# Audio-WestlakeU/SAR-SSL

Hardware: AMD Instinct MI355X
Metric: pretrain_segments_per_sec (higher is better)
Workload: dtype fp16 stem + f32 residual stream (fp16-pair MFMA operands: hi hi + lo hi + hi lo), bf16 backward

## Files before the change

### include/sarssl_hip.h

```cpp
#ifndef SARSSL_HIP_H
#define SARSSL_HIP_H
#ifdef __cplusplus
extern "C" {
#endif

const char* sarssl_last_error(void);
int sarssl_abi_version(void);

typedef struct sarssl_ctx sarssl_ctx;
sarssl_ctx* sarssl_create(int device);
int sarssl_destroy(sarssl_ctx* ctx);
int sarssl_make_current(sarssl_ctx* ctx);
int sarssl_ctx_device(const sarssl_ctx* ctx);
int sarssl_ctx_set_conv_cus(sarssl_ctx* ctx, int ncus);
int sarssl_ctx_fp16_overflow(sarssl_ctx* ctx, int clear, void* stream);
int sarssl_ctx_get_conv_cus(const sarssl_ctx* ctx);
int sarssl_ctx_set_clock_probe(sarssl_ctx* ctx, void* buf);
int sarssl_ctx_attach_step_state(sarssl_ctx* ctx, void* state);
int sarssl_ctx_zero_arena(sarssl_ctx* ctx, const void* base, long bytes);

int sarssl_stft_frontend_pairs(const void* sig, int sig_dtype, int nb, long nsample, int nch, int win_len, int hop, int nfft,
                               int nt, float eps, int pair_mode, float* U, double* magsum, float* out, void* stream);
int sarssl_stft_frontend_pairs_masked(const void* sig, int sig_dtype, int nb, long nsample, int nch, int win_len, int hop, int nfft,
                                      int nt, float eps, int pair_mode, float* U, double* magsum, float* out, const unsigned char* mp,
                                      const int* mch, void* spec, void* spat, int dtype, void* stream);
int sarssl_stft_raw(const void* sig, int sig_dtype, int nb, long nsample, int nch, int win_len, int hop, int nfft, int nt,
                    float* U, double* magsum, float* out, void* stream);
int sarssl_wav_probe(const char* path, int* nch, int* fs, long* nsample);
int sarssl_wav_read_batch(const char* const* paths, int n, long nsample, int nch, int fs, long offset, short* out, int nthreads);
int sarssl_wav_write_batch(const char* const* paths, int n, long nsample, int nch, int fs, const short* in, int nthreads);
int sarssl_mask_sample(unsigned int* mt, int* pos, int nbatch, int npatch, int nmasked, int nmic, long* idx, long* ch);
long sarssl_istft_workspace_bytes(int nb, int nch, int nt);
int sarssl_istft(const float* spec, int nb, int nch, int nt, int win_len, int hop, int nfft, int center, float* frames_ws,
                 float* sig, void* stream);
long sarssl_rir_mix_workspace_bytes(int nb, long ns, int nch, int lmax, int ldmax);
int sarssl_rir_mix(const float* src, const float* rir, const int* rir_len, const float* rir_dp, const int* dp_len, int n0,
                   const float* noise, const float* snr_db, const float* gain, int nb, long ns, int nch, int lmax, int ldmax, void* ws,
                   float* out, void* stream);
long sarssl_diffuse_noise_workspace_bytes(int nb, long ns, int m);
// ... 251 lines not shown
```

### sar-ssl_amd/csrc/api.hip

```cpp
#include "common.h"
#include <stdarg.h>
#include <stdio.h>
#include <stdlib.h>

static thread_local char g_err[512] = "";

void sarssl_set_error(const char* fmt, ...) {
    va_list ap; va_start(ap, fmt); vsnprintf(g_err, sizeof(g_err), fmt, ap); va_end(ap);
}
extern "C" const char* sarssl_last_error() { return g_err; }
extern "C" int sarssl_abi_version() { return 3; }

int sarssl_cu_count() {
    static int cached[64] = {0};
    int dev = 0;
    if (hipGetDevice(&dev) != hipSuccess || dev < 0 || dev >= 64) return 256;
    if (cached[dev] == 0) {
        int n = 0;
        if (hipDeviceGetAttribute(&n, hipDeviceAttributeMultiprocessorCount, dev) != hipSuccess || n <= 0) n = 256;
        cached[dev] = n;
    }
    return cached[dev];
}

// ... 76 lines not shown
extern "C" int sarssl_destroy(sarssl_ctx* ctx) {
    if (ctx && t_ctx == ctx) t_ctx = nullptr;
    if (ctx && ctx->ovf_flag) (void)hipFree(ctx->ovf_flag);
    free(ctx);
    return 0;
}
int* sarssl_overflow_flag() { sarssl_ctx* c = sarssl_current(); return c ? c->ovf_flag : nullptr; }
extern "C" int sarssl_ctx_fp16_overflow(sarssl_ctx* ctx, int clear, void* stream) {
    if (!ctx || !ctx->ovf_flag) return 0;
    int h = 0;
    if (hipMemcpyAsync(&h, ctx->ovf_flag, sizeof(int), hipMemcpyDeviceToHost, (hipStream_t)stream) != hipSuccess) return -1;
    if (clear && hipMemsetAsync(ctx->ovf_flag, 0, sizeof(int), (hipStream_t)stream) != hipSuccess) return -1;
    if (hipStreamSynchronize((hipStream_t)stream) != hipSuccess) return -1;
    return h != 0;
}
extern "C" int sarssl_make_current(sarssl_ctx* ctx) { t_ctx = ctx; return 0; }
extern "C" int sarssl_ctx_device(const sarssl_ctx* ctx) { return ctx ? ctx->device : -1; }
extern "C" int sarssl_ctx_set_conv_cus(sarssl_ctx* ctx, int ncus) {
    SARSSL_REQUIRE(ctx != nullptr, "sarssl_ctx_set_conv_cus");
    ctx->conv_cus_bwd = ncus > 0 ? ncus : 0;
    return 0;
}
extern "C" int sarssl_ctx_get_conv_cus(const sarssl_ctx* ctx) { return ctx ? ctx->conv_cus_bwd : 0; }
extern "C" int sarssl_ctx_set_clock_probe(sarssl_ctx* ctx, void* buf) {
    SARSSL_REQUIRE(ctx != nullptr, "sarssl_ctx_set_clock_probe");
    ctx->conv_clk = (unsigned long long*)buf;
    return 0;
}

int sarssl_mfma_prio() { return 2; }
```

### sar-ssl_amd/csrc/common.h

```cpp
#pragma once
#include <hip/hip_runtime.h>
#include <stdint.h>

typedef __bf16 bf16;
typedef __attribute__((ext_vector_type(8))) __bf16 bf16x8;
typedef __attribute__((ext_vector_type(4))) __bf16 bf16x4;
typedef __attribute__((ext_vector_type(16))) float f32x16;
typedef __attribute__((ext_vector_type(4))) float f32x4;

typedef _Float16 f16;
typedef __attribute__((ext_vector_type(8))) _Float16 f16x8;

enum { SARSSL_F32 = 0, SARSSL_BF16 = 1, SARSSL_I16 = 2, SARSSL_F16 = 3, SARSSL_MIX16 = 4, SARSSL_MIXF32 = 5 };

extern "C" const char* sarssl_last_error();
void sarssl_set_error(const char* fmt, ...);
int sarssl_cu_count();
struct sarssl_ctx {
    int device;
    int conv_cus_bwd;
    unsigned long long* conv_clk;
    const unsigned long long* salt;
    const char* zero_lo; const char* zero_hi;
    int* ovf_flag;
};
int* sarssl_overflow_flag();
sarssl_ctx* sarssl_current();
struct SarsslStepState {
    unsigned long long salt;
    int step;
    float lr, beta1, beta2;
    float step_size;
    float inv_bc2_sqrt;
    int nskipped;
};
int sarssl_mfma_prio();
bool sarssl_prezeroed(const void* p);
#define SARSSL_ZERO(p, bytes, st) (sarssl_prezeroed(p) ? hipSuccess : hipMemsetAsync((p), 0, (bytes), (st)))
const unsigned long long* sarssl_dropout_salt();
#define SARSSL_CHECK_LAUNCH(name)                                          \
    do {                                                                   \
        hipError_t e__ = hipGetLastError();                                \
        if (e__ != hipSuccess) {                                           \
// ... 226 lines not shown
```

### sar-ssl_amd/csrc/gemm.hip

```cpp
#include "gemm_epilogue.h"
#include <stdlib.h>

#define BN 128
#define BK 64
#define PITCH (BK + 8)

template <typename TA, typename TB> struct MfmaT { typedef bf16 type; };
template <> struct MfmaT<f16, f16> { typedef f16 type; };
template <typename T, typename TM>
__device__ __forceinline__ uint4 load_chunk(const T* __restrict__ p, int part) {
    if constexpr (sizeof(T) == 2) return recode8<T, TM>(*(const uint4*)p);
    else { const f8 v = ld8(p); return pack8_part(v, part); }
}

template <typename T, typename TM, bool KC, int ROWS, bool EDGE>
__device__ __forceinline__ void tile_load(const T* __restrict__ p, long ld, int r0, int k0, int R, int Kend, int part, int tid,
                                          uint4 (&regs)[ROWS / 32]) {
    constexpr int CPR = ROWS / 8, KPP = 256 / CPR;
#pragma unroll
    for (int i = 0; i < ROWS / 32; ++i) {
        const T* q = KC ? p + (long)(32 * i) * ld : p + (long)(KPP * i) * ld;
        if constexpr (EDGE) {
            const int gr = KC ? r0 + (tid >> 3) + 32 * i : r0 + (tid % CPR) * 8;
            const int gk = KC ? k0 + (tid & 7) * 8 : k0 + tid / CPR + KPP * i;
            regs[i] = (gr < R && gk < Kend) ? load_chunk<T, TM>(q, part) : make_uint4(0, 0, 0, 0);
        } else regs[i] = load_chunk<T, TM>(q, part);
    }
}
template <bool KC, int ROWS>
__device__ __forceinline__ void tile_store(uint16_t* __restrict__ s, int tid, const uint4 (&regs)[ROWS / 32]) {
    constexpr int CPR = ROWS / 8, KPP = 256 / CPR, PT = ROWS + 32;
#pragma unroll
    for (int i = 0; i < ROWS / 32; ++i) {
        if (KC) *(uint4*)&s[((tid >> 3) + 32 * i) * PITCH + (tid & 7) * 8] = regs[i];
        else *(uint4*)&s[(tid / CPR + KPP * i) * PT + (tid % CPR) * 8] = regs[i];
    }
}

template <int PT>
__device__ __forceinline__ bf16x8 frag_tr(const uint16_t* s, int kbase, int r0, int lane) {
    typedef __attribute__((ext_vector_type(4))) short s16x4;
    const int col = r0 + 16 * ((lane >> 4) & 1) + (lane & 3) * 4;
    union { s16x4 v[2]; bf16x8 b; } u;
#pragma unroll
    for (int h = 0; h < 2; ++h) {
        const int k = kbase + (lane >> 5) * 8 + h * 4 + ((lane & 15) >> 2);
        u.v[h] = __builtin_amdgcn_ds_read_tr16_b64_v4i16((__attribute__((address_space(3))) s16x4*)(s + k * PT + col));
    }
    return u.b;
}

template <typename TA, typename TB, typename TC, bool AKC, bool BKC, int FM, bool EDGE, bool CSUM = false, int NSEG = 0>
__device__ __forceinline__ void gemm_body(const GemmArgs& g, const int bid_x, const int bid_y, const int bid_z, const int grid_x,
                                          const int grid_y, const int grid_z) {
    typedef typename MfmaT<TA, TB>::type TM;
    static_assert(sizeof(TA) == 2 || (sizeof(TA) == 4 && sizeof(TB) == 4), "f32 operands come in pairs (split-bf16 passes)");
    static_assert(NSEG == 0 || ((NSEG == 2 || NSEG == 3) && AKC && BKC && sizeof(TA) == 2 && sizeof(TB) == 2 && FM <= 2), "pair products: NT layout, 16-bit operands");
    constexpr int BM = 64 * FM;
    constexpr int PTA = BM + 32, PTB = BN + 32;
    constexpr int A_ELEMS = AKC ? BM * PITCH : BK * PTA;
    constexpr int B_ELEMS = BKC ? BN * PITCH : BK * PTB;
    constexpr int STAGE = A_ELEMS + B_ELEMS + (NSEG >= 2 ? B_ELEMS : 0) + (NSEG == 3 ? A_ELEMS : 0);
    constexpr int PC = BN + 4;
    constexpr int EPI_ELEMS = 64 * PC * 2;
    constexpr int LDS_ELEMS = STAGE > EPI_ELEMS ? STAGE : EPI_ELEMS;
    __shared__ __attribute__((aligned(16))) uint16_t smem[LDS_ELEMS];
    uint16_t* sA = smem;
    uint16_t* sB = smem + A_ELEMS;
    uint16_t* sB2 = sB + B_ELEMS;
    uint16_t* sA2 = sB2 + B_ELEMS;
    const int tid = threadIdx.x, lane = tid & 63, wave = tid >> 6;
    const int wm = wave >> 1, wn = wave & 1;
    const int nsplit = g.split_k > 0 ? g.split_k : 1;
    const bool slice_major = g.split_k > 0 && ((nsplit & 7) == 0 || nsplit == 4 || nsplit == 2) && grid_z == nsplit;
    const int lin_all = (bid_z * grid_y + bid_y) * grid_x + bid_x;
    const int z = slice_major ? 0 : bid_z / nsplit, ks = slice_major ? lin_all % nsplit : bid_z % nsplit;
    const int z0 = z / g.batch_inner, z1 = z % g.batch_inner;
    const int k_begin = g.split_k > 0 ? ks * g.k_per_split : 0;
    const int k_end = g.split_k > 0 ? min(g.K, k_begin + g.k_per_split) : g.K;
    int bx = bid_x, by = bid_y;
    if (slice_major) {
        const int tile = lin_all / nsplit;
        bx = tile % grid_x; by = tile / grid_x;
    } else if ((grid_y & 7) == 0) {
        const int lin = bid_y * grid_x + bid_x;
        const int xcd = lin & 7, j = lin >> 3;
        by = xcd + 8 * (j / grid_x);
        bx = j % grid_x;
    }
    const int m0 = by * BM, n0 = bx * BN;
    constexpr int CPRA = BM / 8, CPRB = BN / 8;
    const TA* pa = (const TA*)g.A + z0 * g.sA0 + z1 * g.sA1 +
                   (AKC ? (long)(m0 + (tid >> 3)) * g.lda + k_begin + (tid & 7) * 8 : (long)(k_begin + tid / CPRA) * g.lda + m0 + (tid % CPRA) * 8);
    const TB* pb = (const TB*)g.B + z0 * g.sB0 + z1 * g.sB1 +
                   (BKC ? (long)(n0 + (tid >> 3)) * g.ldb + k_begin + (tid & 7) * 8 : (long)(k_begin + tid / CPRB) * g.ldb + n0 + (tid % CPRB) * 8);
    const long stepA = AKC ? BK : (long)BK * g.lda, stepB = BKC ? BK : (long)BK * g.ldb;

    f32x16 acc[FM][2];
#pragma unroll
    for (int i = 0; i < FM; ++i)
#pragma unroll
        for (int j = 0; j < 2; ++j)
#pragma unroll
            for (int r = 0; r < 16; ++r) acc[i][j][r] = 0.f;
    static_assert(!CSUM || FM == 2, "column-sum epilogue: two A fragments share one accumulator");
    const bool do_cs = CSUM && g.csum_ws != nullptr && bx == 0 && wn == 0;
    f32x16 accs;
#pragma unroll
    for (int r = 0; r < 16; ++r) accs[r] = 0.f;
    const uint32_t selw = ((lane & 31) < 16) ? 0x3F803F80u : 0u;

    const int ch = tid & 15, n = n0 + ch * 8;
    float bias8[8];
    if (g.bias && (!EDGE || n + 8 <= g.N)) {
        const float4 b0 = *(const float4*)(g.bias + n), b1 = *(const float4*)(g.bias + n + 4);
        bias8[0] = b0.x; bias8[1] = b0.y; bias8[2] = b0.z; bias8[3] = b0.w; bias8[4] = b1.x; bias8[5] = b1.y; bias8[6] = b1.z; bias8[7] = b1.w;
    } else {
#pragma unroll
        for (int e = 0; e < 8; ++e) bias8[e] = (g.bias && n + e < g.N) ? g.bias[n + e] : 0.f;
    }

    auto mfma_phase = [&](const uint16_t* tA, const uint16_t* tB) {
        auto load_frags = [&](int kk, bf16x8 (&fa)[FM], bf16x8 (&fb)[2]) {
            const int koff = kk * 16 + (lane >> 5) * 8;
#pragma unroll
            for (int i = 0; i < FM; ++i) {
                if (AKC) fa[i] = *(const bf16x8*)&tA[(wm * (FM * 32) + i * 32 + (lane & 31)) * PITCH + koff];
                else fa[i] = frag_tr<PTA>(tA, kk * 16, wm * (FM * 32) + i * 32, lane);
            }
#pragma unroll
            for (int j = 0; j < 2; ++j) {
                if (BKC) fb[j] = *(const bf16x8*)&tB[(wn * 64 + j * 32 + (lane & 31)) * PITCH + koff];
                else fb[j] = frag_tr<PTB>(tB, kk * 16, wn * 64 + j * 32, lane);
            }
        };
        auto mfmas = [&](const bf16x8 (&fa)[FM], const bf16x8 (&fb)[2]) {
#pragma unroll
            for (int i = 0; i < FM; ++i)
#pragma unroll
                for (int j = 0; j < 2; ++j)
                    acc[i][j] = mfma16<TM>(fb[j], fa[i], acc[i][j]);
            if constexpr (CSUM) {
                if (do_cs) {
// ... 2 lines not shown
                    for (int e = 0; e < 4; ++e) { s0.w[e] = selw; s1.w[e] = selw ^ 0x3F803F80u; }
                    accs = __builtin_amdgcn_mfma_f32_32x32x16_bf16(s0.b, fa[0], accs, 0, 0, 0);
                    accs = __builtin_amdgcn_mfma_f32_32x32x16_bf16(s1.b, fa[FM - 1], accs, 0, 0, 0);
                }
            }
        };
        bf16x8 fa0[FM], fb0[2], fa1[FM], fb1[2];
        if (g.prio) __builtin_amdgcn_s_setprio(2);
        load_frags(0, fa0, fb0);
#pragma unroll
        for (int kk = 0; kk < BK / 16; kk += 2) {
            load_frags(kk + 1, fa1, fb1);
            __builtin_amdgcn_sched_barrier(0);
            mfmas(fa0, fb0);
            __builtin_amdgcn_sched_barrier(0);
            if (kk + 2 < BK / 16) load_frags(kk + 2, fa0, fb0);
            __builtin_amdgcn_sched_barrier(0);
            mfmas(fa1, fb1);
            __builtin_amdgcn_sched_barrier(0);
        }
        if (g.prio) __builtin_amdgcn_s_setprio(0);
    };

    if constexpr (NSEG >= 2) {
        const TA* pa2 = (const TA*)g.A2 + (pa - (const TA*)g.A);
        const TB* pb2 = (const TB*)g.B2 + (pb - (const TB*)g.B);
        uint4 ra[BM / 32], rb[BN / 32], rb2[BN / 32], ra2[NSEG == 3 ? BM / 32 : 1];
        auto load_all = [&](int k0) {
            tile_load<TA, TM, AKC, BM, EDGE>(pa, g.lda, m0, k0, g.M, k_end, 0, tid, ra);
            tile_load<TB, TM, BKC, BN, EDGE>(pb, g.ldb, n0, k0, g.N, k_end, 0, tid, rb);
            tile_load<TB, TM, BKC, BN, EDGE>(pb2, g.ldb, n0, k0, g.N, k_end, 0, tid, rb2);
            if constexpr (NSEG == 3) tile_load<TA, TM, AKC, BM, EDGE>(pa2, g.lda, m0, k0, g.M, k_end, 0, tid, ra2);
        };
        auto phase = [&]() {
            auto load_frags = [&](int kk, bf16x8 (&fa)[FM], bf16x8 (&fa2)[FM], bf16x8 (&fb)[2], bf16x8 (&fb2)[2]) {
                const int koff = kk * 16 + (lane >> 5) * 8;
#pragma unroll
                for (int i = 0; i < FM; ++i) {
                    const int o = (wm * (FM * 32) + i * 32 + (lane & 31)) * PITCH + koff;
                    fa[i] = *(const bf16x8*)&sA[o];
                    if constexpr (NSEG == 3) fa2[i] = *(const bf16x8*)&sA2[o];
                }
#pragma unroll
                for (int j = 0; j < 2; ++j) {
                    const int o = (wn * 64 + j * 32 + (lane & 31)) * PITCH + koff;
                    fb[j] = *(const bf16x8*)&sB[o];
                    fb2[j] = *(const bf16x8*)&sB2[o];
                }
            };
            auto mfmas = [&](const bf16x8 (&fa)[FM], const bf16x8 (&fa2)[FM], const bf16x8 (&fb)[2], const bf16x8 (&fb2)[2]) {
#pragma unroll
                for (int i = 0; i < FM; ++i)
#pragma unroll
                    for (int j = 0; j < 2; ++j) acc[i][j] = mfma16<TM>(fb[j], fa[i], acc[i][j]);
#pragma unroll
                for (int i = 0; i < FM; ++i)
#pragma unroll
                    for (int j = 0; j < 2; ++j) acc[i][j] = mfma16<TM>(fb2[j], fa[i], acc[i][j]);
                if constexpr (NSEG == 3) {
#pragma unroll
                    for (int i = 0; i < FM; ++i)
#pragma unroll
                        for (int j = 0; j < 2; ++j) acc[i][j] = mfma16<TM>(fb[j], fa2[i], acc[i][j]);
                }
            };
            bf16x8 fa0[FM], fa20[FM], fb0[2], fb20[2], fa1[FM], fa21[FM], fb1[2], fb21[2];
            if (g.prio) __builtin_amdgcn_s_setprio(2);
            load_frags(0, fa0, fa20, fb0, fb20);
#pragma unroll
            for (int kk = 0; kk < BK / 16; kk += 2) {
                load_frags(kk + 1, fa1, fa21, fb1, fb21);
                __builtin_amdgcn_sched_barrier(0);
                mfmas(fa0, fa20, fb0, fb20);
                __builtin_amdgcn_sched_barrier(0);
                if (kk + 2 < BK / 16) load_frags(kk + 2, fa0, fa20, fb0, fb20);
                __builtin_amdgcn_sched_barrier(0);
                mfmas(fa1, fa21, fb1, fb21);
                __builtin_amdgcn_sched_barrier(0);
            }
            if (g.prio) __builtin_amdgcn_s_setprio(0);
        };
        load_all(k_begin);
        for (int k0 = k_begin; k0 < k_end; k0 += BK) {
            tile_store<AKC, BM>(sA, tid, ra);
            tile_store<BKC, BN>(sB, tid, rb);
            tile_store<BKC, BN>(sB2, tid, rb2);
            if constexpr (NSEG == 3) tile_store<AKC, BM>(sA2, tid, ra2);
            __syncthreads();
            if (k0 + BK < k_end) {
                pa += stepA; pb += stepB; pa2 += stepA; pb2 += stepB;
                load_all(k0 + BK);
            }
            phase();
            __syncthreads();
        }
    } else {
        uint4 ra[BM / 32], rb[BN / 32];
        tile_load<TA, TM, AKC, BM, EDGE>(pa, g.lda, m0, k_begin, g.M, k_end, g.partA, tid, ra);
        tile_load<TB, TM, BKC, BN, EDGE>(pb, g.ldb, n0, k_begin, g.N, k_end, g.partB, tid, rb);
#ifdef GEMM_STAMPS
#define GSTAMP(k) do { if (g.stamps && bid_x == 0 && bid_y == 0 && bid_z == 0 && lane == 0 && kt < 16) g.stamps[((tid >> 6) * 16 + kt) * 8 + (k)] = __builtin_amdgcn_s_memtime(); } while (0)
        int kt = 0;
#else
#define GSTAMP(k) do {} while (0)
#endif
        for (int k0 = k_begin; k0 < k_end; k0 += BK) {
            GSTAMP(0);
            tile_store<AKC, BM>(sA, tid, ra);
            tile_store<BKC, BN>(sB, tid, rb);
            GSTAMP(1);
            __syncthreads();
            GSTAMP(2);
            if (k0 + BK < k_end) {
                pa += stepA; pb += stepB;
                tile_load<TA, TM, AKC, BM, EDGE>(pa, g.lda, m0, k0 + BK, g.M, k_end, g.partA, tid, ra);
                tile_load<TB, TM, BKC, BN, EDGE>(pb, g.ldb, n0, k0 + BK, g.N, k_end, g.partB, tid, rb);
            }
            GSTAMP(3);
            mfma_phase(sA, sB);
            GSTAMP(4);
            __syncthreads();
            GSTAMP(5);
#ifdef GEMM_STAMPS
            ++kt;
#endif
        }
    }

    if constexpr (CSUM) {
        if (do_cs && lane < 32) {
            float* q = g.csum_ws + (long)ks * g.M + m0 + wm * (FM * 32) + lane;
            q[0] = accs[0];
            q[32] = accs[8];
        }
    }
    TC* C = (TC*)g.C + z0 * g.sC0 + z1 * g.sC1;
    const TC* Rz = g.resid ? (const TC*)g.resid + z0 * g.sR0 + z1 * g.sR1 : nullptr;
    TC* P = g.preact ? (TC*)g.preact + z0 * g.sC0 + z1 * g.sC1 : nullptr;
    const TC* Xa = g.aux ? (const TC*)g.aux + z0 * g.sC0 + z1 * g.sC1 : nullptr;
    float* W = g.acc_ws ? g.acc_ws + (long)z * g.M * g.N : nullptr;
    float* Wp = (g.split_k > 0) ? g.acc_ws + ((long)z * nsplit + ks) * g.M * g.N : nullptr;
    const bool vec_ok = ((g.N & 7) == 0) && ((g.ldc & 7) == 0) && (!g.resid || (g.ldr & 7) == 0);
    DropCtx dc;
    dc.init(g);
    float* sC = (float*)smem;
    const TC* Ex = (!EDGE && sizeof(TC) == 2 && g.split_k <= 0 && !g.acc_out) ? (Rz && !Xa ? Rz : (Xa && !Rz ? Xa : nullptr)) : nullptr;
    const long ldex = (Ex == Rz) ? g.ldr : g.ldc;
    const bool ex_f16 = g.aux_f16 && Ex == Xa && Ex != nullptr;
    f8 exa[4], exb[4];
    auto load_ex = [&](int i, f8 (&dst)[4]) {
#pragma unroll
// ... 20 lines not shown
            const int m = m0 + (r >> 5) * (FM * 32) + i * 32 + (r & 31);
            if (EDGE && (m >= g.M || n >= g.N)) continue;
            f8 v;
            const float4 a0 = *(const float4*)&sC[r * PC + ch * 8], a1 = *(const float4*)&sC[r * PC + ch * 8 + 4];
            v.v[0] = g.alpha * a0.x; v.v[1] = g.alpha * a0.y; v.v[2] = g.alpha * a0.z; v.v[3] = g.alpha * a0.w;
            v.v[4] = g.alpha * a1.x; v.v[5] = g.alpha * a1.y; v.v[6] = g.alpha * a1.z; v.v[7] = g.alpha * a1.w;
            epilogue8<TC, EDGE>(g, v, z, m, n, C, Rz, P, Xa, W, Wp, bias8, vec_ok, dc, has_ex, cur[k]);
        }
        if (i + 1 < FM) __syncthreads();
    };
    slice(0, exa, exb);
    if constexpr (FM >= 2) slice(1, exb, exa);
    if constexpr (FM >= 4) { slice(2, exa, exb); slice(3, exb, exa); }
}

#ifdef GEMM_STAMPS
static unsigned long long* g_gemm_stamps_host = nullptr;
extern "C" int sarssl_gemm_stamp_buffer(void* p) { g_gemm_stamps_host = (unsigned long long*)p; return 0; }
#endif
template <typename TA, typename TB, typename TC, bool AKC, bool BKC, int FM, bool EDGE>
__global__ __launch_bounds__(256) __attribute__((amdgpu_waves_per_eu(FM == 4 ? 2 : 3))) void gemm_kernel(GemmArgs g) {
    gemm_body<TA, TB, TC, AKC, BKC, FM, EDGE>(g, blockIdx.x, blockIdx.y, blockIdx.z, gridDim.x, gridDim.y, gridDim.z);
}
template <typename TC, int FM, bool EDGE, int NSEG>
__global__ __launch_bounds__(256) __attribute__((amdgpu_waves_per_eu(2))) void gemm_seg_kernel(GemmArgs g) {
    gemm_body<f16, f16, TC, true, true, FM, EDGE, false, NSEG>(g, blockIdx.x, blockIdx.y, blockIdx.z, gridDim.x, gridDim.y, gridDim.z);
}

#define GROUP_MAXP 12
struct GemmGroup {
    GemmArgs p[GROUP_MAXP];
    int gx[GROUP_MAXP], gy[GROUP_MAXP], first[GROUP_MAXP + 1];
    int n;
};
template <typename TB>
__global__ __launch_bounds__(256) __attribute__((amdgpu_waves_per_eu(3))) void gemm_group_tn_kernel(GemmGroup a) {
    int q = 0;
    while (q + 1 < a.n && (int)blockIdx.x >= a.first[q + 1]) ++q;
    const int local = blockIdx.x - a.first[q];
    const int gx = a.gx[q], gy = a.gy[q], ns = a.p[q].split_k;
    if (local >= gx * gy * ns) return;
    const int bz = local / (gx * gy), rem = local - bz * (gx * gy);
    gemm_body<bf16, TB, float, false, false, 2, false, true>(a.p[q], rem % gx, rem / gx, bz, gx, gy, ns);
}

__global__ void splitk_reduce_kernel(const float* __restrict__ ws, int nsplit, int M, int N, float* __restrict__ C, long ldc,
                                     int batch_inner, long sC0, long sC1) {
    const long mn = (long)M * N;
    const int z = blockIdx.y;
// ... 185 lines not shown
            const int npass = precise ? 3 : 1;
            for (int pass = 0; pass < npass; ++pass) {
                p.partA = precise ? (pass == 1) : 0; p.partB = precise ? (pass == 0) : 0;
                int rc = launch_layout<float, float, float, false>(p, a_kc, b_kc, nbatch, st); if (rc) return rc;
                rc = reduce(); if (rc) return rc;
            }
            return 0;
        }
        if (!precise) return launch_layout<float, float, float, false>(g, a_kc, b_kc, nbatch, st);
        SARSSL_REQUIRE(ws != nullptr, "sarssl_gemm(precise needs workspace)");
        g.acc_ws = ws;
        GemmArgs p = g;
        p.partA = 0; p.partB = 1; p.acc_in = 0; p.acc_out = 1;
        int rc = launch_layout<float, float, float, false>(p, a_kc, b_kc, nbatch, st); if (rc) return rc;
        p.partA = 1; p.partB = 0; p.acc_in = 1; p.acc_out = 1;
        rc = launch_layout<float, float, float, false>(p, a_kc, b_kc, nbatch, st); if (rc) return rc;
        p.partA = 0; p.partB = 0; p.acc_in = 1; p.acc_out = 0;
        return launch_layout<float, float, float, false>(p, a_kc, b_kc, nbatch, st);
    }
    sarssl_set_error("sarssl_gemm: unsupported dtype combination (%d,%d,%d)", dtA, dtB, dtC);
    return -1;
}

template <typename TC, int NSEG>
static int launch_seg(const GemmArgs& g, hipStream_t st) {
    const long wg2 = (long)((g.M + 127) / 128) * ((g.N + BN - 1) / BN);
    const long cus = sarssl_cu_count();
    int fm = (g.M >= 128 && (wg2 <= cus || (wg2 <= 2 * cus && g.K <= 256))) ? 1 : 2;
#ifdef SARSSL_PROBE_ENV
    { static const int force_fm = [] { const char* e = getenv("SARSSL_SPLIT_FM"); return e ? atoi(e) : 0; }(); if (force_fm) fm = force_fm; }
#endif
    const int bm = 64 * fm;
    const bool vec_ok = ((g.N & 7) == 0) && ((g.ldc & 7) == 0) && (!g.resid || (g.ldr & 7) == 0);
    const bool edge = (g.M % bm) != 0 || (g.N % BN) != 0 || (g.K % BK) != 0 || !vec_ok;
    dim3 grid((g.N + BN - 1) / BN, (g.M + bm - 1) / bm, 1);
    if (fm == 1) { if (edge) gemm_seg_kernel<TC, 1, true, NSEG><<<grid, 256, 0, st>>>(g); else gemm_seg_kernel<TC, 1, false, NSEG><<<grid, 256, 0, st>>>(g); }
    else { if (edge) gemm_seg_kernel<TC, 2, true, NSEG><<<grid, 256, 0, st>>>(g); else gemm_seg_kernel<TC, 2, false, NSEG><<<grid, 256, 0, st>>>(g); }
    SARSSL_CHECK_LAUNCH("sarssl_gemm_split");
    return 0;
}
extern "C" int sarssl_gemm_split(const void* A, const void* A_lo, const void* B, const void* B_lo, void* C, int dtC, int M, int N, int K,
                                 long lda, long ldb, long ldc, float out_scale, const float* bias, int act, const void* resid, long ldr,
                                 float res_scale, void* preact, float p_drop, unsigned long long seed, void* stream) {
    SARSSL_REQUIRE(M > 0 && N > 0 && K > 0 && A && B && C, "sarssl_gemm_split");
    SARSSL_REQUIRE(K % 8 == 0 && lda % 8 == 0 && ldb % 8 == 0, "sarssl_gemm_split(alignment)");
    SARSSL_REQUIRE(dtC == SARSSL_F16 || dtC == SARSSL_F32, "sarssl_gemm_split(dtC)");
    GemmArgs g;
    g.A = A; g.B = B; g.C = C; g.M = M; g.N = N; g.K = K; g.lda = lda; g.ldb = ldb; g.ldc = ldc;
    g.batch_inner = 1; g.sA0 = g.sA1 = g.sB0 = g.sB1 = g.sC0 = g.sC1 = 0;
    g.alpha = 1.f; g.out_scale = out_scale; g.bias = bias; g.act = act;
    g.resid = resid; g.ldr = ldr; g.sR0 = g.sR1 = 0; g.res_scale = res_scale;
    g.preact = preact; g.aux = nullptr; g.aux_act = 0; g.aux_f16 = 0; g.acc_ws = nullptr; g.acc_in = 0; g.acc_out = 0; g.partA = 0; g.partB = 0;
    g.p_drop = p_drop; g.seed = seed; g.salt = sarssl_dropout_salt(); g.prio = (sarssl_mfma_prio() == 1 || sarssl_mfma_prio() == 3);
    g.split_k = 0; g.k_per_split = K; g.row_shift = 0; g.csum_ws = nullptr;
    SARSSL_REQUIRE(!A_lo || B_lo, "sarssl_gemm_split(A_lo needs B_lo)");
    if (A_lo && B_lo) { g.A2 = A_lo; g.B2 = B_lo; g.nseg = 3; }
    else if (B_lo) { g.A2 = nullptr; g.B2 = B_lo; g.nseg = 2; }
    else { g.A2 = nullptr; g.B2 = nullptr; g.nseg = 1; }
#ifdef GEMM_STAMPS
    g.stamps = nullptr;
#endif
    hipStream_t st = (hipStream_t)stream;
    if (g.nseg == 1) {
        if (dtC == SARSSL_F16) return launch_layout<f16, f16, f16, true>(g, 1, 1, 1, st);
        return launch_layout<f16, f16, float, false>(g, 1, 1, 1, st);
    }
    if (g.nseg == 2) return dtC == SARSSL_F16 ? launch_seg<f16, 2>(g, st) : launch_seg<float, 2>(g, st);
    return dtC == SARSSL_F16 ? launch_seg<f16, 3>(g, st) : launch_seg<float, 3>(g, st);
}

extern "C" int sarssl_gemm_group_tn(const void* const* A, const void* const* B, float* const* ws, const int* M, const int* N,
                                    const int* K, const long* lda, const long* ldb, const int* split_k, int* split_out,
                                    float* const* csum_ws, int n_prob, int dtB, void* stream) {
    SARSSL_REQUIRE(n_prob > 0 && n_prob <= GROUP_MAXP && (dtB == SARSSL_BF16 || dtB == SARSSL_F16), "sarssl_gemm_group_tn");
    GemmGroup a;
    a.n = n_prob;
    int total = 0;
    bool edge = false;
    for (int q = 0; q < n_prob; ++q) {
        SARSSL_REQUIRE(M[q] > 0 && N[q] > 0 && K[q] > 0 && split_k[q] > 0 && M[q] % 8 == 0 && N[q] % 8 == 0 && lda[q] % 8 == 0 &&
                       ldb[q] % 8 == 0 && ws[q] != nullptr, "sarssl_gemm_group_tn(shape)");
        const int per = ((K[q] + split_k[q] - 1) / split_k[q] + BK - 1) / BK * BK;
        const int ns = (K[q] + per - 1) / per;
// ... 22 lines not shown
```

### sar-ssl_amd/hip.py

```python
import ctypes
import os

import torch

from . import _lib
from ._lib import c_void_p, c_int, c_long, c_float, c_ulonglong

F32, BF16, I16, F16, MIX16, MIXF32 = 0, 1, 2, 3, 4, 5
_DT = {torch.float32: F32, torch.bfloat16: BF16, torch.int16: I16, torch.float16: F16}
_16 = (torch.bfloat16, torch.float16)


def dt(t):
    return _DT[t.dtype]


def dt_ga(g, a):
    if a is None or g.dtype == a.dtype:
        return _DT[g.dtype]
    if g.dtype == torch.bfloat16 and a.dtype == torch.float16:
        return MIX16
    if g.dtype == torch.bfloat16 and a.dtype == torch.float32:
        return MIXF32
    raise _lib.SarsslHipError("unsupported gradient / saved-activation dtype pair (%s, %s)" % (g.dtype, a.dtype))
# ... 950 lines not shown


_stamps = None


def stamp(label):
    if _stamps is None:
        return
    buf, labels = _stamps
    i = len(labels)
    if i < buf.numel():
        labels.append(label)
        _lib.call("sarssl_stamp", c_void_p(buf.data_ptr() + 8 * i), _stream())


def conv_clock_probe(buf):
    _lib.call("sarssl_ctx_set_clock_probe", c_void_p(_lib._make_current()), _p(buf))


def conv_cus_override(ncus):
    _lib.call("sarssl_ctx_set_conv_cus", c_void_p(_lib._make_current()), c_int(int(ncus)))


def _wgrad_part(B, F, T, device):
    nbytes = _lib.lib().sarssl_conv3x3_wgrad_workspace_bytes
    nbytes.restype = c_long
    return workspace(nbytes(c_int(B), c_int(F), c_int(T)), device, "wgrad_part")


def conv3x3_wgrad_c1(dy, a0, W1, scale, shift, acc_into):
    _need_cuda(dy, a0, W1)
    B, F, T, _ = a0.shape
    assert a0.dtype in _16 and dy.dtype == torch.bfloat16 and acc_into.shape == (64, 64, 3, 3) and acc_into.is_contiguous()
    part = _wgrad_part(B, F, T, a0.device)
    with _Timed("conv3x3_wgrad_kernel"):
        _lib.call("sarssl_conv3x3_wgrad_c1_acc", _p(dy), _p(a0), _p(W1), c_int(B), c_int(F), c_int(T), _p(scale), _p(shift), _p(acc_into),
                  _p(part), c_int(dt(a0)), _stream())
    return True


def conv3x3_wgrad_c4(y3, dy4, W4, aff3, train, red, y2, scale, shift, acc_into, out=None, pgrads=None):
    _need_cuda(y3, dy4, W4, aff3, red, y2)
    B, F, T, C = y3.shape
    assert C == 64 and y3.dtype in _16 and y2.dtype == y3.dtype and y2.shape == y3.shape and dy4.dtype == torch.bfloat16
    assert dy4.shape == (B, T, F, 4) and dy4.is_contiguous() and y3.is_contiguous() and y2.is_contiguous() and W4.is_contiguous()
    assert aff3.dtype == torch.float32 and aff3.is_contiguous() and aff3.numel() == 256 and red.numel() == 384
# ... 686 lines not shown
```

Baseline: 6011.

## Add shallow K-tile variant for fp16 pair-product GEMMs with scalarised addressing

Adds a KB=32 K-depth template path for the split-precision (hi/lo pair) GEMM kernels, used by default when K < 1024 and overridable per context. It brings a new K-row swizzle, loads that use a wave-uniform base pointer plus a 32-bit per-lane offset, a bias load moved after the main loop, and a higher waves-per-EU target. The goal is to cut LDS and register footprint, raising occupancy and reducing address arithmetic for short-K GEMMs. The cost is more K iterations with barriers, plus a new stride limit on lda and ldb.

```diff
diff --git a/include/sarssl_hip.h b/include/sarssl_hip.h
--- a/include/sarssl_hip.h
+++ b/include/sarssl_hip.h
@@ -15,6 +15,7 @@
 int sarssl_ctx_set_conv_cus(sarssl_ctx* ctx, int ncus);
 int sarssl_ctx_fp16_overflow(sarssl_ctx* ctx, int clear, void* stream);
 int sarssl_ctx_get_conv_cus(const sarssl_ctx* ctx);
+int sarssl_ctx_set_pair_kdepth(sarssl_ctx* ctx, int depth);
 int sarssl_ctx_set_clock_probe(sarssl_ctx* ctx, void* buf);
 int sarssl_ctx_attach_step_state(sarssl_ctx* ctx, void* state);
 int sarssl_ctx_zero_arena(sarssl_ctx* ctx, const void* base, long bytes);
diff --git a/sar-ssl_amd/csrc/api.hip b/sar-ssl_amd/csrc/api.hip
--- a/sar-ssl_amd/csrc/api.hip
+++ b/sar-ssl_amd/csrc/api.hip
@@ -122,6 +122,11 @@
     return 0;
 }
 extern "C" int sarssl_ctx_get_conv_cus(const sarssl_ctx* ctx) { return ctx ? ctx->conv_cus_bwd : 0; }
+extern "C" int sarssl_ctx_set_pair_kdepth(sarssl_ctx* ctx, int depth) {
+    SARSSL_REQUIRE(ctx != nullptr && (depth == 0 || depth == 32 || depth == 64), "sarssl_ctx_set_pair_kdepth");
+    ctx->pair_kdepth = depth;
+    return 0;
+}
 extern "C" int sarssl_ctx_set_clock_probe(sarssl_ctx* ctx, void* buf) {
     SARSSL_REQUIRE(ctx != nullptr, "sarssl_ctx_set_clock_probe");
     ctx->conv_clk = (unsigned long long*)buf;
diff --git a/sar-ssl_amd/csrc/common.h b/sar-ssl_amd/csrc/common.h
--- a/sar-ssl_amd/csrc/common.h
+++ b/sar-ssl_amd/csrc/common.h
@@ -19,6 +19,7 @@
 struct sarssl_ctx {
     int device;
     int conv_cus_bwd;
+    int pair_kdepth;
     unsigned long long* conv_clk;
     const unsigned long long* salt;
     const char* zero_lo; const char* zero_hi;
diff --git a/sar-ssl_amd/csrc/gemm.hip b/sar-ssl_amd/csrc/gemm.hip
--- a/sar-ssl_amd/csrc/gemm.hip
+++ b/sar-ssl_amd/csrc/gemm.hip
@@ -13,26 +13,49 @@
     else { const f8 v = ld8(p); return pack8_part(v, part); }
 }
 
-template <typename T, typename TM, bool KC, int ROWS, bool EDGE>
+template <int KB> __device__ __forceinline__ int krow(int t) {
+    if constexpr (KB == 64) return t >> 3;
+    else { const int q = t >> 2; return (q & ~7) | ((q & 1) << 2) | ((q >> 1) & 3); }
+}
+template <typename T, typename TM, bool KC, int ROWS, bool EDGE, int KB = BK>
 __device__ __forceinline__ void tile_load(const T* __restrict__ p, long ld, int r0, int k0, int R, int Kend, int part, int tid,
-                                          uint4 (&regs)[ROWS / 32]) {
-    constexpr int CPR = ROWS / 8, KPP = 256 / CPR;
-#pragma unroll
-    for (int i = 0; i < ROWS / 32; ++i) {
-        const T* q = KC ? p + (long)(32 * i) * ld : p + (long)(KPP * i) * ld;
+                                          uint4 (&regs)[ROWS * KB / 2048]) {
+    constexpr int CPR = ROWS / 8, KPP = 256 / CPR, RPP = 2048 / KB;
+#pragma unroll
+    for (int i = 0; i < ROWS * KB / 2048; ++i) {
+        const T* q = KC ? p + (long)(RPP * i) * ld : p + (long)(KPP * i) * ld;
         if constexpr (EDGE) {
-            const int gr = KC ? r0 + (tid >> 3) + 32 * i : r0 + (tid % CPR) * 8;
-            const int gk = KC ? k0 + (tid & 7) * 8 : k0 + tid / CPR + KPP * i;
+            const int gr = KC ? r0 + krow<KB>(tid) + RPP * i : r0 + (tid % CPR) * 8;
+            const int gk = KC ? k0 + (tid & (KB / 8 - 1)) * 8 : k0 + tid / CPR + KPP * i;
             regs[i] = (gr < R && gk < Kend) ? load_chunk<T, TM>(q, part) : make_uint4(0, 0, 0, 0);
         } else regs[i] = load_chunk<T, TM>(q, part);
     }
 }
-template <bool KC, int ROWS>
-__device__ __forceinline__ void tile_store(uint16_t* __restrict__ s, int tid, const uint4 (&regs)[ROWS / 32]) {
-    constexpr int CPR = ROWS / 8, KPP = 256 / CPR, PT = ROWS + 32;
-#pragma unroll
-    for (int i = 0; i < ROWS / 32; ++i) {
-        if (KC) *(uint4*)&s[((tid >> 3) + 32 * i) * PITCH + (tid & 7) * 8] = regs[i];
+template <int ROWS, bool EDGE, int KB>
+__device__ __forceinline__ void tile_load_u(const char* __restrict__ base, uint32_t voff, long ld, int r0, int k0, int R, int Kend, int tid,
+                                            uint4 (&regs)[ROWS * KB / 2048]) {
+    constexpr int RPP = 2048 / KB;
+#pragma unroll
+    for (int i = 0; i < ROWS * KB / 2048; ++i) {
+        const uint64_t bi = (uint64_t)(base + (long)(RPP * i) * ld * 2);
+        const char* sb = (const char*)(((uint64_t)(uint32_t)__builtin_amdgcn_readfirstlane((int)(bi >> 32)) << 32) |
+                                       (uint32_t)__builtin_amdgcn_readfirstlane((int)(uint32_t)bi));
+        typedef uint32_t u32x4 __attribute__((ext_vector_type(4)));
+        typedef const __attribute__((address_space(1))) u32x4* gptr;
+        u32x4 v = {0u, 0u, 0u, 0u};
+        if constexpr (EDGE) {
+            const int gr = r0 + krow<KB>(tid) + RPP * i, gk = k0 + (tid & (KB / 8 - 1)) * 8;
+            if (gr < R && gk < Kend) v = *(gptr)(sb + voff);
+        } else v = *(gptr)(sb + voff);
+        regs[i] = make_uint4(v.x, v.y, v.z, v.w);
+    }
+}
+template <bool KC, int ROWS, int KB = BK>
+__device__ __forceinline__ void tile_store(uint16_t* __restrict__ s, int tid, const uint4 (&regs)[ROWS * KB / 2048]) {
+    constexpr int CPR = ROWS / 8, KPP = 256 / CPR, PT = ROWS + 32, RPP = 2048 / KB;
+#pragma unroll
+    for (int i = 0; i < ROWS * KB / 2048; ++i) {
+        if (KC) *(uint4*)&s[(krow<KB>(tid) + RPP * i) * (KB + 8) + (tid & (KB / 8 - 1)) * 8] = regs[i];
         else *(uint4*)&s[(tid / CPR + KPP * i) * PT + (tid % CPR) * 8] = regs[i];
     }
 }
@@ -50,16 +73,18 @@
     return u.b;
 }
 
-template <typename TA, typename TB, typename TC, bool AKC, bool BKC, int FM, bool EDGE, bool CSUM = false, int NSEG = 0>
+template <typename TA, typename TB, typename TC, bool AKC, bool BKC, int FM, bool EDGE, bool CSUM = false, int NSEG = 0, int KB = BK>
 __device__ __forceinline__ void gemm_body(const GemmArgs& g, const int bid_x, const int bid_y, const int bid_z, const int grid_x,
                                           const int grid_y, const int grid_z) {
     typedef typename MfmaT<TA, TB>::type TM;
     static_assert(sizeof(TA) == 2 || (sizeof(TA) == 4 && sizeof(TB) == 4), "f32 operands come in pairs (split-bf16 passes)");
     static_assert(NSEG == 0 || ((NSEG == 2 || NSEG == 3) && AKC && BKC && sizeof(TA) == 2 && sizeof(TB) == 2 && FM <= 2), "pair products: NT layout, 16-bit operands");
+    static_assert(KB == BK || (KB == 32 && NSEG >= 2), "the shallow K-tile exists for the pair products only");
     constexpr int BM = 64 * FM;
     constexpr int PTA = BM + 32, PTB = BN + 32;
-    constexpr int A_ELEMS = AKC ? BM * PITCH : BK * PTA;
-    constexpr int B_ELEMS = BKC ? BN * PITCH : BK * PTB;
+    constexpr int PK = KB + 8;
+    constexpr int A_ELEMS = AKC ? BM * PK : BK * PTA;
+    constexpr int B_ELEMS = BKC ? BN * PK : BK * PTB;
     constexpr int STAGE = A_ELEMS + B_ELEMS + (NSEG >= 2 ? B_ELEMS : 0) + (NSEG == 3 ? A_ELEMS : 0);
     constexpr int PC = BN + 4;
     constexpr int EPI_ELEMS = 64 * PC * 2;
@@ -91,10 +116,10 @@
     const int m0 = by * BM, n0 = bx * BN;
     constexpr int CPRA = BM / 8, CPRB = BN / 8;
     const TA* pa = (const TA*)g.A + z0 * g.sA0 + z1 * g.sA1 +
-                   (AKC ? (long)(m0 + (tid >> 3)) * g.lda + k_begin + (tid & 7) * 8 : (long)(k_begin + tid / CPRA) * g.lda + m0 + (tid % CPRA) * 8);
+                   (AKC ? (long)(m0 + krow<KB>(tid)) * g.lda + k_begin + (tid & (KB / 8 - 1)) * 8 : (long)(k_begin + tid / CPRA) * g.lda + m0 + (tid % CPRA) * 8);
     const TB* pb = (const TB*)g.B + z0 * g.sB0 + z1 * g.sB1 +
-                   (BKC ? (long)(n0 + (tid >> 3)) * g.ldb + k_begin + (tid & 7) * 8 : (long)(k_begin + tid / CPRB) * g.ldb + n0 + (tid % CPRB) * 8);
-    const long stepA = AKC ? BK : (long)BK * g.lda, stepB = BKC ? BK : (long)BK * g.ldb;
+                   (BKC ? (long)(n0 + krow<KB>(tid)) * g.ldb + k_begin + (tid & (KB / 8 - 1)) * 8 : (long)(k_begin + tid / CPRB) * g.ldb + n0 + (tid % CPRB) * 8);
+    const long stepA = AKC ? KB : (long)BK * g.lda, stepB = BKC ? KB : (long)BK * g.ldb;
 
     f32x16 acc[FM][2];
 #pragma unroll
@@ -112,13 +137,16 @@
 
     const int ch = tid & 15, n = n0 + ch * 8;
     float bias8[8];
-    if (g.bias && (!EDGE || n + 8 <= g.N)) {
-        const float4 b0 = *(const float4*)(g.bias + n), b1 = *(const float4*)(g.bias + n + 4);
-        bias8[0] = b0.x; bias8[1] = b0.y; bias8[2] = b0.z; bias8[3] = b0.w; bias8[4] = b1.x; bias8[5] = b1.y; bias8[6] = b1.z; bias8[7] = b1.w;
-    } else {
-#pragma unroll
-        for (int e = 0; e < 8; ++e) bias8[e] = (g.bias && n + e < g.N) ? g.bias[n + e] : 0.f;
-    }
+    auto load_bias = [&]() {
+        if (g.bias && (!EDGE || n + 8 <= g.N)) {
+            const float4 b0 = *(const float4*)(g.bias + n), b1 = *(const float4*)(g.bias + n + 4);
+            bias8[0] = b0.x; bias8[1] = b0.y; bias8[2] = b0.z; bias8[3] = b0.w; bias8[4] = b1.x; bias8[5] = b1.y; bias8[6] = b1.z; bias8[7] = b1.w;
+        } else {
+#pragma unroll
+            for (int e = 0; e < 8; ++e) bias8[e] = (g.bias && n + e < g.N) ? g.bias[n + e] : 0.f;
+        }
+    };
+    if constexpr (KB == BK) load_bias();
 
     auto mfma_phase = [&](const uint16_t* tA, const uint16_t* tB) {
         auto load_frags = [&](int kk, bf16x8 (&fa)[FM], bf16x8 (&fb)[2]) {
@@ -167,88 +195,141 @@
         if (g.prio) __builtin_amdgcn_s_setprio(0);
     };
 
+#ifdef GEMM_STAMPS
+#define GSTAMP(k) do { if (g.stamps && bid_x == 0 && bid_y == 0 && bid_z == 0 && lane == 0 && kt < 16) g.stamps[((tid >> 6) * 16 + kt) * 8 + (k)] = __builtin_amdgcn_s_memtime(); } while (0)
+#define GSTAMP_KT int kt = 0
+#define GSTAMP_NEXT ++kt
+#else
+#define GSTAMP(k) do {} while (0)
+#define GSTAMP_KT do {} while (0)
+#define GSTAMP_NEXT do {} while (0)
+#endif
     if constexpr (NSEG >= 2) {
         const TA* pa2 = (const TA*)g.A2 + (pa - (const TA*)g.A);
         const TB* pb2 = (const TB*)g.B2 + (pb - (const TB*)g.B);
-        uint4 ra[BM / 32], rb[BN / 32], rb2[BN / 32], ra2[NSEG == 3 ? BM / 32 : 1];
+        constexpr int NA = BM * KB / 2048, NB = BN * KB / 2048;
+        uint4 ra[NA], rb[NB], rb2[NB], ra2[NSEG == 3 ? NA : 1];
+        const char* uA = (const char*)((const TA*)g.A + (long)m0 * g.lda + k_begin);
+        const char* uB = (const char*)((const TB*)g.B + (long)n0 * g.ldb + k_begin);
+        const char* uA2 = (const char*)((const TA*)g.A2 + (long)m0 * g.lda + k_begin);
+        const char* uB2 = (const char*)((const TB*)g.B2 + (long)n0 * g.ldb + k_begin);
+        const uint32_t vA = ((uint32_t)krow<KB>(tid) * (uint32_t)g.lda + (tid & (KB / 8 - 1)) * 8) * 2u;
+        const uint32_t vB = ((uint32_t)krow<KB>(tid) * (uint32_t)g.ldb + (tid & (KB / 8 - 1)) * 8) * 2u;
         auto load_all = [&](int k0) {
-            tile_load<TA, TM, AKC, BM, EDGE>(pa, g.lda, m0, k0, g.M, k_end, 0, tid, ra);
-            tile_load<TB, TM, BKC, BN, EDGE>(pb, g.ldb, n0, k0, g.N, k_end, 0, tid, rb);
-            tile_load<TB, TM, BKC, BN, EDGE>(pb2, g.ldb, n0, k0, g.N, k_end, 0, tid, rb2);
-            if constexpr (NSEG == 3) tile_load<TA, TM, AKC, BM, EDGE>(pa2, g.lda, m0, k0, g.M, k_end, 0, tid, ra2);
+            if constexpr (KB == BK) {
+                tile_load<TA, TM, AKC, BM, EDGE>(pa, g.lda, m0, k0, g.M, k_end, 0, tid, ra);
+                tile_load<TB, TM, BKC, BN, EDGE>(pb, g.ldb, n0, k0, g.N, k_end, 0, tid, rb);
+                tile_load<TB, TM, BKC, BN, EDGE>(pb2, g.ldb, n0, k0, g.N, k_end, 0, tid, rb2);
+                if constexpr (NSEG == 3) tile_load<TA, TM, AKC, BM, EDGE>(pa2, g.lda, m0, k0, g.M, k_end, 0, tid, ra2);
+            } else {
+                tile_load_u<BM, EDGE, KB>(uA, vA, g.lda, m0, k0, g.M, k_end, tid, ra);
+                tile_load_u<BN, EDGE, KB>(uB, vB, g.ldb, n0, k0, g.N, k_end, tid, rb);
+                tile_load_u<BN, EDGE, KB>(uB2, vB, g.ldb, n0, k0, g.N, k_end, tid, rb2);
+                if constexpr (NSEG == 3) tile_load_u<BM, EDGE, KB>(uA2, vA, g.lda, m0, k0, g.M, k_end, tid, ra2);
+            }
+        };
+        const int oa = (wm * (FM * 32) + (lane & 31)) * PK + (lane >> 5) * 8, ob = (wn * 64 + (lane & 31)) * PK + (lane >> 5) * 8;
+        auto load_hi = [&](int kk, bf16x8 (&fa)[FM], bf16x8 (&fb)[2]) {
+#pragma unroll
+            for (int i = 0; i < FM; ++i) fa[i] = *(const bf16x8*)&sA[oa + i * 32 * PK + kk * 16];
+#pragma unroll
+            for (int j = 0; j < 2; ++j) fb[j] = *(const bf16x8*)&sB[ob + j * 32 * PK + kk * 16];
+        };
+        auto load_lo = [&](int kk, bf16x8 (&fa2)[FM], bf16x8 (&fb2)[2]) {
+#pragma unroll
+            for (int j = 0; j < 2; ++j) fb2[j] = *(const bf16x8*)&sB2[ob + j * 32 * PK + kk * 16];
+            if constexpr (NSEG == 3) {
+#pragma unroll
+                for (int i = 0; i < FM; ++i) fa2[i] = *(const bf16x8*)&sA2[oa + i * 32 * PK + kk * 16];
+            }
+        };
+        auto mfmas = [&](const bf16x8 (&fa)[FM], const bf16x8 (&fa2)[FM], const bf16x8 (&fb)[2], const bf16x8 (&fb2)[2]) {
+#pragma unroll
+            for (int i = 0; i < FM; ++i)
+#pragma unroll
+                for (int j = 0; j < 2; ++j) acc[i][j] = mfma16<TM>(fb[j], fa[i], acc[i][j]);
+#pragma unroll
+            for (int i = 0; i < FM; ++i)
+#pragma unroll
+                for (int j = 0; j < 2; ++j) acc[i][j] = mfma16<TM>(fb2[j], fa[i], acc[i][j]);
+            if constexpr (NSEG == 3) {
+#pragma unroll
+                for (int i = 0; i < FM; ++i)
+#pragma unroll
+                    for (int j = 0; j < 2; ++j) acc[i][j] = mfma16<TM>(fb[j], fa2[i], acc[i][j]);
+            }
         };
         auto phase = [&]() {
-            auto load_frags = [&](int kk, bf16x8 (&fa)[FM], bf16x8 (&fa2)[FM], bf16x8 (&fb)[2], bf16x8 (&fb2)[2]) {
-                const int koff = kk * 16 + (lane >> 5) * 8;
-#pragma unroll
-                for (int i = 0; i < FM; ++i) {
-                    const int o = (wm * (FM * 32) + i * 32 + (lane & 31)) * PITCH + koff;
-                    fa[i] = *(const bf16x8*)&sA[o];
-                    if constexpr (NSEG == 3) fa2[i] = *(const bf16x8*)&sA2[o];
+            if (g.prio) __builtin_amdgcn_s_setprio(2);
+            if constexpr (KB == BK) {
+                auto load_frags = [&](int kk, bf16x8 (&fa)[FM], bf16x8 (&fa2)[FM], bf16x8 (&fb)[2], bf16x8 (&fb2)[2]) {
+#pragma unroll
+                    for (int i = 0; i < FM; ++i) {
+                        fa[i] = *(const bf16x8*)&sA[oa + i * 32 * PK + kk * 16];
+                        if constexpr (NSEG == 3) fa2[i] = *(const bf16x8*)&sA2[oa + i * 32 * PK + kk * 16];
+                    }
+#pragma unroll
+                    for (int j = 0; j < 2; ++j) {
+                        fb[j] = *(const bf16x8*)&sB[ob + j * 32 * PK + kk * 16];
+                        fb2[j] = *(const bf16x8*)&sB2[ob + j * 32 * PK + kk * 16];
+                    }
+                };
+                bf16x8 fa0[FM], fa20[FM], fb0[2], fb20[2], fa1[FM], fa21[FM], fb1[2], fb21[2];
+                load_frags(0, fa0, fa20, fb0, fb20);
+#pragma unroll
+                for (int kk = 0; kk < KB / 16; kk += 2) {
+                    load_frags(kk + 1, fa1, fa21, fb1, fb21);
+                    __builtin_amdgcn_sched_barrier(0);
+                    mfmas(fa0, fa20, fb0, fb20);
+                    __builtin_amdgcn_sched_barrier(0);
+                    if (kk + 2 < KB / 16) load_frags(kk + 2, fa0, fa20, fb0, fb20);
+                    __builtin_amdgcn_sched_barrier(0);
+                    mfmas(fa1, fa21, fb1, fb21);
+                    __builtin_amdgcn_sched_barrier(0);
                 }
-#pragma unroll
-                for (int j = 0; j < 2; ++j) {
-                    const int o = (wn * 64 + j * 32 + (lane & 31)) * PITCH + koff;
-                    fb[j] = *(const bf16x8*)&sB[o];
-                    fb2[j] = *(const bf16x8*)&sB2[o];
-                }
-            };
-            auto mfmas = [&](const bf16x8 (&fa)[FM], const bf16x8 (&fa2)[FM], const bf16x8 (&fb)[2], const bf16x8 (&fb2)[2]) {
-#pragma unroll
-                for (int i = 0; i < FM; ++i)
-#pragma unroll
-                    for (int j = 0; j < 2; ++j) acc[i][j] = mfma16<TM>(fb[j], fa[i], acc[i][j]);
-#pragma unroll
-                for (int i = 0; i < FM; ++i)
-#pragma unroll
-                    for (int j = 0; j < 2; ++j) acc[i][j] = mfma16<TM>(fb2[j], fa[i], acc[i][j]);
-                if constexpr (NSEG == 3) {
-#pragma unroll
-                    for (int i = 0; i < FM; ++i)
-#pragma unroll
-                        for (int j = 0; j < 2; ++j) acc[i][j] = mfma16<TM>(fb[j], fa2[i], acc[i][j]);
-                }
-            };
-            bf16x8 fa0[FM], fa20[FM], fb0[2], fb20[2], fa1[FM], fa21[FM], fb1[2], fb21[2];
-            if (g.prio) __builtin_amdgcn_s_setprio(2);
-            load_frags(0, fa0, fa20, fb0, fb20);
-#pragma unroll
-            for (int kk = 0; kk < BK / 16; kk += 2) {
-                load_frags(kk + 1, fa1, fa21, fb1, fb21);
+            } else {
+                bf16x8 fa0[FM], fb0[2], fa1[FM], fb1[2], fa2[FM], fb2[2];
+                load_hi(0, fa0, fb0); load_lo(0, fa2, fb2);
                 __builtin_amdgcn_sched_barrier(0);
-                mfmas(fa0, fa20, fb0, fb20);
+                load_hi(1, fa1, fb1);
                 __builtin_amdgcn_sched_barrier(0);
-                if (kk + 2 < BK / 16) load_frags(kk + 2, fa0, fa20, fb0, fb20);
+                mfmas(fa0, fa2, fb0, fb2);
                 __builtin_amdgcn_sched_barrier(0);
-                mfmas(fa1, fa21, fb1, fb21);
+                load_lo(1, fa2, fb2);
+                __builtin_amdgcn_sched_barrier(0);
+                mfmas(fa1, fa2, fb1, fb2);
                 __builtin_amdgcn_sched_barrier(0);
             }
             if (g.prio) __builtin_amdgcn_s_setprio(0);
         };
         load_all(k_begin);
-        for (int k0 = k_begin; k0 < k_end; k0 += BK) {
-            tile_store<AKC, BM>(sA, tid, ra);
-            tile_store<BKC, BN>(sB, tid, rb);
-            tile_store<BKC, BN>(sB2, tid, rb2);
-            if constexpr (NSEG == 3) tile_store<AKC, BM>(sA2, tid, ra2);
+        GSTAMP_KT;
+        for (int k0 = k_begin; k0 < k_end; k0 += KB) {
+            GSTAMP(0);
+            tile_store<AKC, BM, KB>(sA, tid, ra);
+            tile_store<BKC, BN, KB>(sB, tid, rb);
+            tile_store<BKC, BN, KB>(sB2, tid, rb2);
+            if constexpr (NSEG == 3) tile_store<AKC, BM, KB>(sA2, tid, ra2);
+            GSTAMP(1);
             __syncthreads();
-            if (k0 + BK < k_end) {
-                pa += stepA; pb += stepB; pa2 += stepA; pb2 += stepB;
-                load_all(k0 + BK);
-            }
+            GSTAMP(2);
+            if (k0 + KB < k_end) {
+                if constexpr (KB == BK) { pa += stepA; pb += stepB; pa2 += stepA; pb2 += stepB; }
+                else { uA += KB * 2; uB += KB * 2; uA2 += KB * 2; uB2 += KB * 2; }
+                load_all(k0 + KB);
+            }
+            GSTAMP(3);
             phase();
+            GSTAMP(4);
             __syncthreads();
+            GSTAMP(5);
+            GSTAMP_NEXT;
         }
     } else {
         uint4 ra[BM / 32], rb[BN / 32];
         tile_load<TA, TM, AKC, BM, EDGE>(pa, g.lda, m0, k_begin, g.M, k_end, g.partA, tid, ra);
         tile_load<TB, TM, BKC, BN, EDGE>(pb, g.ldb, n0, k_begin, g.N, k_end, g.partB, tid, rb);
-#ifdef GEMM_STAMPS
-#define GSTAMP(k) do { if (g.stamps && bid_x == 0 && bid_y == 0 && bid_z == 0 && lane == 0 && kt < 16) g.stamps[((tid >> 6) * 16 + kt) * 8 + (k)] = __builtin_amdgcn_s_memtime(); } while (0)
-        int kt = 0;
-#else
-#define GSTAMP(k) do {} while (0)
-#endif
+        GSTAMP_KT;
         for (int k0 = k_begin; k0 < k_end; k0 += BK) {
             GSTAMP(0);
             tile_store<AKC, BM>(sA, tid, ra);
@@ -266,12 +347,11 @@
             GSTAMP(4);
             __syncthreads();
             GSTAMP(5);
-#ifdef GEMM_STAMPS
-            ++kt;
-#endif
-        }
-    }
-
+            GSTAMP_NEXT;
+        }
+    }
+
+    if constexpr (KB != BK) load_bias();
     if constexpr (CSUM) {
         if (do_cs && lane < 32) {
             float* q = g.csum_ws + (long)ks * g.M + m0 + wm * (FM * 32) + lane;
@@ -338,9 +418,9 @@
 __global__ __launch_bounds__(256) __attribute__((amdgpu_waves_per_eu(FM == 4 ? 2 : 3))) void gemm_kernel(GemmArgs g) {
     gemm_body<TA, TB, TC, AKC, BKC, FM, EDGE>(g, blockIdx.x, blockIdx.y, blockIdx.z, gridDim.x, gridDim.y, gridDim.z);
 }
-template <typename TC, int FM, bool EDGE, int NSEG>
-__global__ __launch_bounds__(256) __attribute__((amdgpu_waves_per_eu(2))) void gemm_seg_kernel(GemmArgs g) {
-    gemm_body<f16, f16, TC, true, true, FM, EDGE, false, NSEG>(g, blockIdx.x, blockIdx.y, blockIdx.z, gridDim.x, gridDim.y, gridDim.z);
+template <typename TC, int FM, bool EDGE, int NSEG, int KB>
+__global__ __launch_bounds__(256) __attribute__((amdgpu_waves_per_eu(KB == 32 ? 3 : 2))) void gemm_seg_kernel(GemmArgs g) {
+    gemm_body<f16, f16, TC, true, true, FM, EDGE, false, NSEG, KB>(g, blockIdx.x, blockIdx.y, blockIdx.z, gridDim.x, gridDim.y, gridDim.z);
 }
 
 #define GROUP_MAXP 12
@@ -572,6 +652,12 @@
     return -1;
 }
 
+template <typename TC, int NSEG, int KB>
+static void launch_seg_kb(const GemmArgs& g, int fm, bool edge, dim3 grid, hipStream_t st) {
+    if (fm == 1) { if (edge) gemm_seg_kernel<TC, 1, true, NSEG, KB><<<grid, 256, 0, st>>>(g); else gemm_seg_kernel<TC, 1, false, NSEG, KB><<<grid, 256, 0, st>>>(g); }
+    else { if (edge) gemm_seg_kernel<TC, 2, true, NSEG, KB><<<grid, 256, 0, st>>>(g); else gemm_seg_kernel<TC, 2, false, NSEG, KB><<<grid, 256, 0, st>>>(g); }
+}
+static int pair_kdepth_rule(const GemmArgs& g) { return g.K >= 1024 ? BK : 32; }
 template <typename TC, int NSEG>
 static int launch_seg(const GemmArgs& g, hipStream_t st) {
     const long wg2 = (long)((g.M + 127) / 128) * ((g.N + BN - 1) / BN);
@@ -580,12 +666,14 @@
 #ifdef SARSSL_PROBE_ENV
     { static const int force_fm = [] { const char* e = getenv("SARSSL_SPLIT_FM"); return e ? atoi(e) : 0; }(); if (force_fm) fm = force_fm; }
 #endif
+    const sarssl_ctx* cx = sarssl_current();
+    const int kb = (cx && cx->pair_kdepth) ? cx->pair_kdepth : pair_kdepth_rule(g);
     const int bm = 64 * fm;
     const bool vec_ok = ((g.N & 7) == 0) && ((g.ldc & 7) == 0) && (!g.resid || (g.ldr & 7) == 0);
-    const bool edge = (g.M % bm) != 0 || (g.N % BN) != 0 || (g.K % BK) != 0 || !vec_ok;
+    const bool edge = (g.M % bm) != 0 || (g.N % BN) != 0 || (g.K % kb) != 0 || !vec_ok;
     dim3 grid((g.N + BN - 1) / BN, (g.M + bm - 1) / bm, 1);
-    if (fm == 1) { if (edge) gemm_seg_kernel<TC, 1, true, NSEG><<<grid, 256, 0, st>>>(g); else gemm_seg_kernel<TC, 1, false, NSEG><<<grid, 256, 0, st>>>(g); }
-    else { if (edge) gemm_seg_kernel<TC, 2, true, NSEG><<<grid, 256, 0, st>>>(g); else gemm_seg_kernel<TC, 2, false, NSEG><<<grid, 256, 0, st>>>(g); }
+    if (kb == 32) launch_seg_kb<TC, NSEG, 32>(g, fm, edge, grid, st);
+    else launch_seg_kb<TC, NSEG, BK>(g, fm, edge, grid, st);
     SARSSL_CHECK_LAUNCH("sarssl_gemm_split");
     return 0;
 }
@@ -594,6 +682,7 @@
                                  float res_scale, void* preact, float p_drop, unsigned long long seed, void* stream) {
     SARSSL_REQUIRE(M > 0 && N > 0 && K > 0 && A && B && C, "sarssl_gemm_split");
     SARSSL_REQUIRE(K % 8 == 0 && lda % 8 == 0 && ldb % 8 == 0, "sarssl_gemm_split(alignment)");
+    SARSSL_REQUIRE(lda > 0 && ldb > 0 && lda < (1L << 24) && ldb < (1L << 24), "sarssl_gemm_split(row strides)");
     SARSSL_REQUIRE(dtC == SARSSL_F16 || dtC == SARSSL_F32, "sarssl_gemm_split(dtC)");
     GemmArgs g;
     g.A = A; g.B = B; g.C = C; g.M = M; g.N = N; g.K = K; g.lda = lda; g.ldb = ldb; g.ldc = ldc;
@@ -608,7 +697,7 @@
     else if (B_lo) { g.A2 = nullptr; g.B2 = B_lo; g.nseg = 2; }
     else { g.A2 = nullptr; g.B2 = nullptr; g.nseg = 1; }
 #ifdef GEMM_STAMPS
-    g.stamps = nullptr;
+    g.stamps = g_gemm_stamps_host;
 #endif
     hipStream_t st = (hipStream_t)stream;
     if (g.nseg == 1) {
diff --git a/sar-ssl_amd/hip.py b/sar-ssl_amd/hip.py
--- a/sar-ssl_amd/hip.py
+++ b/sar-ssl_amd/hip.py
@@ -996,6 +996,10 @@
     _lib.call("sarssl_ctx_set_conv_cus", c_void_p(_lib._make_current()), c_int(int(ncus)))
 
 
+def pair_kdepth_override(depth):
+    _lib.call("sarssl_ctx_set_pair_kdepth", c_void_p(_lib._make_current()), c_int(int(depth)))
+
+
 def _wgrad_part(B, F, T, device):
     nbytes = _lib.lib().sarssl_conv3x3_wgrad_workspace_bytes
     nbytes.restype = c_long
```

Result: faster. 6075, median of 6 (+1.1%).
